# lionl1106/Clip-Neural-image-conpression

Measured on AMD Instinct MI355X. Metric: images/sec @256px 50-step DDIM, batch=8/GPU, higher is better.
Workload: dtype bf16; 1 GPU; 256px base=128 ch_mult=(1, 2, 2) 50-step DDIM (eta=0), batch=8/GPU, key-seeded synthetic weights (out.* x0.1), synthetic z / x_T; global_batch=8, parallelism=dp1 (independent batches, no collective in the loop), graph=hipGraph, one replay per step, steps_in_flight=1

## Files before the change

clip-neural-image-conpression_amd/csrc/ccn_api.hip:

```cpp
#include "../../include/ccn_hip.h"
#include "ccn_internal.h"

#include <algorithm>
#include <cmath>
#include <cstdio>
#include <cstdlib>
#include <cstring>
#include <functional>
#include <map>
#include <memory>
#include <string>
#include <vector>

using namespace ccn;

namespace {

thread_local std::string g_err;
int fail(int code, const std::string& msg) { g_err = msg; return code; }
#define HIPCHK(expr)                                                                                     \
    do {                                                                                                 \
        hipError_t e_ = (expr);                                                                          \
        if (e_ != hipSuccess)                                                                            \
            return fail(CCN_EHIP, std::string(#expr) + ": " + hipGetErrorString(e_));                    \
// ... 87 lines not shown
    std::vector<int32_t> ts;
    std::vector<float> coef;
    std::vector<float> sigma;
    const float* noise = nullptr;
    hipGraph_t graph = nullptr;
    hipGraphExec_t exec = nullptr;
};

struct RouteRec {
    std::string name;
    int kind = 0;
    const char* kernel = "";
    int th = 0, ksplit = 1, n_nt = 1;
    const char* gn = "none";
    bool film = false, res = false;
    int ops = -1;
};

constexpr size_t kMaxGraphsPerPlan = 4;
struct Plan {
    int B = 0, H = 0, W = 0, steps = 0;
    void* ws = nullptr;
    size_t bytes = 0;
    int32_t* ts_dev = nullptr;
    float *temb = nullptr, *t1 = nullptr, *tp = nullptr, *zp = nullptr, *film = nullptr;
    float *zbuf = nullptr, *xstate = nullptr;
    std::vector<std::pair<void*, size_t>> zero_once;
    unsigned* counters = nullptr;
    int n_counters = 0;
    std::vector<int32_t> ts_keep;
    std::vector<Launch> ops;
    std::map<std::string, TensorRef> named;
    std::vector<RouteRec> routes;
    std::vector<GraphEntry> graphs;
    ~Plan() {
        for (auto& g : graphs) {
            if (g.exec) (void)hipGraphExecDestroy(g.exec);
            if (g.graph) (void)hipGraphDestroy(g.graph);
        }
    }
};

}

struct ccn_handle_s {
// ... 346 lines not shown
        a.in = in.p; a.w = cw.w; a.wfrag = r.uses_frag() ? cw.wfrag : nullptr; a.bias = cw.bias; a.out = out.p;
        a.film = nullptr; a.res = res ? res->p : nullptr;
        a.ops = cw.split ? 1 : 0; a.wscale_inv = cw.inv_scale;
        RouteRec rec;
        if (h->split) rec.ops = a.ops;
        rec.kind = cw.kind; rec.th = r.th; rec.ksplit = r.ksplit; rec.n_nt = r.n_nt; rec.film = film_off >= 0; rec.res = res != nullptr;
        rec.gn = gn_ab ? "prologue" : "none";
        static const bool no_instat = diag_env("CCN_NO_INSTAT") != nullptr;
        if (in_norm) {
            const int G_in = groups_for(cw.Cin), cpg_in = cw.Cin / G_in;
            if (r.gs_ok && !no_instat && in.C == cw.Cin && conv_in_kernel_stats(h->cfg.dtype, in.C, G_in, in.n_sp, in.bn)) {
                a.gs_part = in.part; a.gs_gamma = in_norm->gamma; a.gs_beta = in_norm->beta;
                a.gs_inv_count = 1.0 / ((double)cpg_in * in.H * in.W);
                a.gs_nsp = in.n_sp; a.gs_nnt = in.n_nt; a.gs_bn = in.bn; a.gs_cpg = cpg_in;
                rec.gn = "instat";
            } else { gn_ab = gn(in, *in_norm); rec.gn = "prologue"; }
        }
        a.gn_ab = gn_ab;
        rec.kernel = conv_kernel_name(conv_kernel_for(cw.kind, cw.BN, a));
        plan->routes.push_back(rec);
        if (r.ksplit == 2) {
            a.kpart = bump.take((size_t)B * g.Hout * g.Wout * cw.Cout * h->elem);
            const size_t fbytes = (size_t)B * r.fin_blocks * 4 * sizeof(unsigned);
            a.kflag = (unsigned*)bump.take(fbytes);
            if (a.kflag) plan->zero_once.push_back({a.kflag, fbytes});
        }
        a.film_bstride = film_stride;
        a.err = h->err_dev;
        if (want_part) {
            out.part = (float2*)bump.take((size_t)B * a.G * a.nslot * sizeof(float2));
            out.n_sp = r.part_nsp; out.n_nt = r.part_nnt; out.bn = r.part_bn;
// ... 88 lines not shown
        return o;
    }

    TensorRef resblock(const ResW& r, const TensorRef& x, bool out_feeds_gn, int film_off = -2)
    {
        static const bool preact_pr = diag_env("CCN_PREACT_PR") != nullptr;
        const bool pre = conv_wants_preact(r.c1.kind, r.c1.BN, r.c1.Cout_pad / r.c1.BN) && r.C / (h->elem == 2 ? 8 : 4) <= 256 &&
                         (preact_pr || r.c1.Cout_pad / r.c1.BN >= 6 || !route(r.c1, x.H, x.W, false, false, false).pr);
        static const bool fuse_act = !diag_env("CCN_NO_FUSED_GNACT");
        const bool f1 = pre && fuse_act && x.n_sp > 0, f2 = pre && fuse_act;
        TensorRef y = new_tensor(r.C, x.H, x.W);
        if (f1) { TensorRef xa = preact_fused(x, r.n1); conv(r.c1, F_C3S1, xa, y, nullptr, film_off == -2 ? r.film_off : film_off, nullptr, true); }
        else if (pre) {
            const float2* ab1 = gn(x, r.n1);
            TensorRef xa = preact(x, ab1); conv(r.c1, F_C3S1, xa, y, nullptr, film_off == -2 ? r.film_off : film_off, nullptr, true);
        } else conv(r.c1, F_C3S1, x, y, nullptr, film_off == -2 ? r.film_off : film_off, nullptr, true, false, false, &r.n1);
        label(r.prefix + ".film", f1 ? "preact_fused" : (pre ? "preact" : nullptr));
        plan->named[r.prefix + ".film"] = y;
        TensorRef o = new_tensor(r.C, x.H, x.W);
        if (f2) { TensorRef ya = preact_fused(y, r.n2); conv(r.c2, F_C3S1, ya, o, nullptr, -1, &x, out_feeds_gn); }
        else if (pre) {
            const float2* ab2 = gn(y, r.n2);
            TensorRef ya = preact(y, ab2); conv(r.c2, F_C3S1, ya, o, nullptr, -1, &x, out_feeds_gn);
        } else conv(r.c2, F_C3S1, y, o, nullptr, -1, &x, out_feeds_gn, false, false, &r.n2);
        label(r.prefix, f2 ? "preact_fused" : (pre ? "preact" : nullptr));
        plan->named[r.prefix] = o;
        return o;
    }
};

int build_plan(ccn_handle_s* h, Plan* plan, void* ws, bool measure)
{
    const ccn_config_t& c = h->cfg;
    PlanBuilder pb(h, plan, ws, measure);
    const int B = plan->B, H = plan->H, W = plan->W, S = plan->steps;
    const int TR = B > S ? B : S, FR = S * B > B ? S * B : B;
    plan->ts_dev = (int32_t*)pb.bump.take((size_t)S * 4);
    plan->temb = (float*)pb.bump.take((size_t)TR * c.time_dim * 4);
    plan->t1 = (float*)pb.bump.take((size_t)TR * c.time_dim * 4 * 4);
    plan->tp = (float*)pb.bump.take((size_t)TR * c.time_dim * 4);
    plan->zp = (float*)pb.bump.take((size_t)B * c.time_dim * 4);
    plan->film = (float*)pb.bump.take((size_t)FR * h->F * 4);
    plan->zbuf = (float*)pb.bump.take((size_t)B * c.z_dim * 4);
    plan->xstate = (float*)pb.bump.take((size_t)B * c.img_ch * H * W * 4);
    plan->counters = (unsigned*)pb.bump.take((size_t)kMaxNorms * B * 4);
    plan->n_counters = 0;

    plan->ops.clear(); plan->named.clear(); plan->routes.clear();
    TensorRef img; img.C = c.img_ch; img.H = H; img.W = W;
    TensorRef x;
    std::vector<TensorRef> skips;
    const size_t nl = h->layers.size();
    for (size_t li = 0; li < nl; ++li) {
        const Layer& L = h->layers[li];
        const bool next_is_gn = li + 1 < nl && (h->layers[li + 1].type == L_RES || h->layers[li + 1].type == L_HEAD);
        switch (L.type) {
            case L_STEM: {
                x = pb.new_tensor(h->stem.Cout, H, W);
                pb.conv(h->stem, F_STEM, img, x, nullptr, -1, nullptr, next_is_gn, true, false);
                pb.label(L.name);
                plan->named[L.name] = x;
                break;
            }
// ... 18 lines not shown
                TensorRef sk = skips.back(); skips.pop_back();
                if (sk.C != cw.Cout || sk.H != o.H || sk.W != o.W) return fail(CCN_EINVAL, "skip shape mismatch");
                pb.conv(cw, F_CT4, x, o, nullptr, -1, &sk, next_is_gn);
                pb.label(L.name);
                plan->named[L.name] = o;
                x = o;
                break;
            }
            case L_HEAD: {
                static const bool no_head2 = diag_env("CCN_NO_HEAD2") != nullptr;
                if (!no_head2 && head2_supported(c.dtype, h->head.Cin, h->head.Cout, h->G)) {
                    std::shared_ptr<ConvArgs> ap(new ConvArgs());
                    ConvArgs& a = *ap;
                    a.in = x.p; a.bias = h->head.bias; a.B = B; a.Hin = H; a.Win = W; a.Cin = h->head.Cin; a.Cout = h->head.Cout;
                    a.Hout = H; a.Wout = W;
                    const float2* ab = pb.gn(x, h->out_norm);
                    void* scratch = pb.bump.take(head2_scratch_bytes(B, x.C));
                    const float* wf = h->head_w_f32;
                    const double macs = (double)B * H * W * h->head.Cout * 9.0 * h->head.Cin;
                    Launch Lh{F_HEAD, 2.0 * macs, ((double)B * H * W * x.C + 9.0 * x.C * h->head.Cout) * h->elem + 3.0 * (double)B * H * W * h->head.Cout * 4, nullptr};
                    Lh.fn = [=](hipStream_t s, const StepCtx& sc) -> hipError_t {
                        ConvArgs k = *ap;
                        k.x_state = sc.x_state; k.eps_out = sc.eps_out; k.do_ddim = sc.do_ddim;
                        k.c0 = sc.c[0]; k.c1 = sc.c[1]; k.c2 = sc.c[2]; k.c3 = sc.c[3];
                        k.noise = sc.noise; k.sigma = sc.sigma;
                        return launch_head2(k, ab, wf, scratch, sc.step, s);
                    };
                    plan->ops.push_back(std::move(Lh));
                    RouteRec rec;
                    rec.name = L.name; rec.kind = KIND_HEAD; rec.kernel = "head2"; rec.th = 8; rec.gn = "weights";
                    if (h->split) rec.ops = 0;
                    plan->routes.push_back(rec);
                    break;
                }
                const float2* ab = pb.gn(x, h->out_norm);
                TensorRef none;
                pb.conv(h->head, F_HEAD, x, none, ab, -1, nullptr, false, false, true);
                pb.label(L.name);
                break;
            }
        }
    }
    plan->bytes = align_up(pb.bump.off, 256);
    return CCN_OK;
}

void drop_plans(ccn_handle_s* h, size_t keep_newest)
{
    if (h->plans.size() <= keep_newest) return;
    (void)hipDeviceSynchronize();
    while (h->plans.size() > keep_newest) h->plans.erase(h->plans.begin());
}

// ... 55 lines not shown
    if (h->profiling) {
        int rc = ensure_events(h, h->ev_used + 2);
        if (rc) return rc;
        const int e0 = (int)h->ev_used, e1 = e0 + 1;
        h->ev_used += 2;
        HIPCHK(hipEventRecord(h->ev_pool[e0], s));
        HIPCHK(L.fn(s, c));
        HIPCHK(hipEventRecord(h->ev_pool[e1], s));
        h->recs.push_back({L.family, L.flops, L.bytes, e0, e1});
        return CCN_OK;
    }
    HIPCHK(L.fn(s, c));
    return CCN_OK;
}

int run_conditioning(ccn_handle_s* h, Plan* p, hipStream_t s, const int64_t* t_i64, int TR, int FR, int a_div)
{
    const ccn_config_t& c = h->cfg;
    const int td = c.time_dim, B = p->B;
    std::vector<Launch> v;
    const float* z = p->zbuf;
    v.push_back({F_COND, 0, 0, [=](hipStream_t st, const StepCtx&) {
        return t_i64 ? launch_temb_i64(t_i64, p->temb, TR, td, st) : launch_temb_i32(p->ts_dev, p->temb, TR, td, st); }});
    v.push_back({F_COND, 2.0 * TR * td * 4.0 * td, 0, [=](hipStream_t st, const StepCtx&) {
        return launch_linear(p->temb, nullptr, 1, TR, h->tp0_w, h->tp0_b, p->t1, TR, td, 4 * td, 1, st); }});
    v.push_back({F_COND, 2.0 * TR * td * 4.0 * td, 0, [=](hipStream_t st, const StepCtx&) {
        return launch_linear(p->t1, nullptr, 1, TR, h->tp2_w, h->tp2_b, p->tp, TR, 4 * td, td, 0, st); }});
    v.push_back({F_COND, 2.0 * B * c.z_dim * td, 0, [=](hipStream_t st, const StepCtx&) {
        return launch_linear(z, nullptr, 1, B, h->zp_w, h->zp_b, p->zp, B, c.z_dim, td, 1, st); }});
    v.push_back({F_COND, 2.0 * FR * td * (double)h->F, 0, [=](hipStream_t st, const StepCtx&) {
        return launch_linear(p->tp, p->zp, a_div, B, h->film_w, h->film_b, p->film, FR, td, h->F, 0, st); }});
    StepCtx c0;
    for (auto& L : v) { int rc = run_launch(h, L, s, c0); if (rc) return rc; }
    return CCN_OK;
}

int run_steps(ccn_handle_s* h, Plan* p, hipStream_t s, int steps, const float* coef, const float* sigma = nullptr, const float* noise = nullptr)
{
    const size_t img = (size_t)p->B * h->cfg.img_ch * p->H * p->W;
    for (int i = 0; i < steps; ++i) {
        StepCtx c;
        c.step = i; c.x_in = p->xstate; c.x_state = p->xstate; c.eps_out = nullptr; c.do_ddim = 1;
        for (int k = 0; k < 4; ++k) c.c[k] = coef[i * 4 + k];
        if (sigma && noise && sigma[i] > 0.f) { c.noise = noise + (size_t)i * img; c.sigma = sigma[i]; }
        for (auto& L : p->ops) { int rc = run_launch(h, L, s, c); if (rc) return rc; }
    }
// ... 240 lines not shown
    if (rc) return rc;
    *bytes = p.bytes;
    return CCN_OK;
}

int ccn_forward(ccn_handle_t h, const float* x_dev, const float* z_dev, const int64_t* t_dev, float* eps_dev,
                int32_t B, int32_t H, int32_t W, void* workspace_dev, size_t workspace_bytes, void* stream)
{
    int rc = check_ready(h);
    if (rc) return rc;
    if (!x_dev || !z_dev || !t_dev || !eps_dev) return fail(CCN_EINVAL, "null tensor pointer");
    Plan* p = nullptr;
    if ((rc = get_plan(h, B, H, W, 1, workspace_dev, workspace_bytes, &p))) return rc;
    hipStream_t s = (hipStream_t)stream;
    HIPCHK(hipMemcpyAsync(p->zbuf, z_dev, (size_t)B * h->cfg.z_dim * 4, hipMemcpyDeviceToDevice, s));
    if ((rc = run_conditioning(h, p, s, t_dev, B, B, 1))) return rc;
    StepCtx c;
    c.step = 0; c.x_in = x_dev; c.x_state = nullptr; c.eps_out = eps_dev; c.do_ddim = 0;
    for (auto& L : p->ops) if ((rc = run_launch(h, L, s, c))) return rc;
    return CCN_OK;
}

static int sample_impl(ccn_handle_t h, const float* z_dev, const float* x_T_dev, float* x_out_dev, int32_t B, int32_t H, int32_t W,
                       int32_t steps, const int32_t* ts_host, const float* coef_host, const float* sigma_host, const float* noise_dev,
                       void* workspace_dev, size_t workspace_bytes, void* stream, int32_t use_graph)
{
    int rc = check_ready(h);
    if (rc) return rc;
    if (!z_dev || !x_T_dev || !x_out_dev || !ts_host || !coef_host) return fail(CCN_EINVAL, "null pointer");
    Plan* p = nullptr;
    if ((rc = get_plan(h, B, H, W, steps, workspace_dev, workspace_bytes, &p))) return rc;
    hipStream_t s = (hipStream_t)stream;
    const size_t img_bytes = (size_t)B * h->cfg.img_ch * H * W * 4;
    HIPCHK(hipMemcpyAsync(p->zbuf, z_dev, (size_t)B * h->cfg.z_dim * 4, hipMemcpyDeviceToDevice, s));
    if (x_T_dev != p->xstate) HIPCHK(hipMemcpyAsync(p->xstate, x_T_dev, img_bytes, hipMemcpyDeviceToDevice, s));

    if (p->ts_keep.size() != (size_t)steps || std::memcmp(p->ts_keep.data(), ts_host, (size_t)steps * 4)) {
        HIPCHK(hipStreamSynchronize(s));
        p->ts_keep.assign(ts_host, ts_host + steps);
        HIPCHK(hipMemcpy(p->ts_dev, p->ts_keep.data(), (size_t)steps * 4, hipMemcpyHostToDevice));
    }
    if (use_graph && !h->profiling) {
        GraphEntry* ge = nullptr;
        for (auto& g : p->graphs)
            if (g.steps == steps && !std::memcmp(g.ts.data(), ts_host, (size_t)steps * 4) &&
                !std::memcmp(g.coef.data(), coef_host, (size_t)steps * 16) && g.noise == noise_dev &&
                g.sigma.size() == (sigma_host ? (size_t)steps : 0) &&
                (!sigma_host || !std::memcmp(g.sigma.data(), sigma_host, (size_t)steps * 4))) { ge = &g; break; }
        if (!ge) {
            GraphEntry g;
            g.steps = steps; g.ts.assign(ts_host, ts_host + steps); g.coef.assign(coef_host, coef_host + steps * 4);
            if (sigma_host) g.sigma.assign(sigma_host, sigma_host + steps);
            g.noise = noise_dev;
            HIPCHK(hipStreamBeginCapture(h->cap_stream, hipStreamCaptureModeRelaxed));
            rc = run_conditioning(h, p, h->cap_stream, nullptr, steps, steps * B, B);
            if (!rc) rc = run_steps(h, p, h->cap_stream, steps, coef_host, sigma_host, noise_dev);
            hipGraph_t graph = nullptr;
            const hipError_t ce = hipStreamEndCapture(h->cap_stream, &graph);
            if (rc) { if (graph) (void)hipGraphDestroy(graph); return rc; }
            if (ce != hipSuccess) return fail(CCN_EHIP, std::string("hipStreamEndCapture: ") + hipGetErrorString(ce));
            g.graph = graph;
            HIPCHK(hipGraphInstantiate(&g.exec, g.graph, nullptr, nullptr, 0));
            if (p->graphs.size() >= kMaxGraphsPerPlan) {
                HIPCHK(hipDeviceSynchronize());
                GraphEntry& old = p->graphs.front();
                if (old.exec) (void)hipGraphExecDestroy(old.exec);
                if (old.graph) (void)hipGraphDestroy(old.graph);
                p->graphs.erase(p->graphs.begin());
            }
            p->graphs.push_back(g);
            ge = &p->graphs.back();
        } else if (ge != &p->graphs.back()) {
            std::rotate(p->graphs.begin() + (ge - p->graphs.data()), p->graphs.begin() + (ge - p->graphs.data()) + 1, p->graphs.end());
            ge = &p->graphs.back();
        }
        HIPCHK(hipGraphLaunch(ge->exec, s));
    } else {
        if ((rc = run_conditioning(h, p, s, nullptr, steps, steps * B, B))) return rc;
        if ((rc = run_steps(h, p, s, steps, coef_host, sigma_host, noise_dev))) return rc;
    }
    if (x_out_dev != p->xstate) HIPCHK(hipMemcpyAsync(x_out_dev, p->xstate, img_bytes, hipMemcpyDeviceToDevice, s));
    return CCN_OK;
}

int ccn_sample(ccn_handle_t h, const float* z_dev, const float* x_T_dev, float* x_out_dev, int32_t B, int32_t H, int32_t W,
               int32_t steps, const int32_t* ts_host, const float* coef_host, void* workspace_dev, size_t workspace_bytes,
               void* stream, int32_t use_graph)
{
    return sample_impl(h, z_dev, x_T_dev, x_out_dev, B, H, W, steps, ts_host, coef_host, nullptr, nullptr, workspace_dev, workspace_bytes, stream, use_graph);
}

int ccn_sample_eta(ccn_handle_t h, const float* z_dev, const float* x_T_dev, float* x_out_dev, int32_t B, int32_t H, int32_t W,
                   int32_t steps, const int32_t* ts_host, const float* coef_host, const float* sigma_host, const float* noise_dev,
// ... 102 lines not shown
    const TensorRef& t = it->second;
    if (out_elems < (size_t)p->B * t.C * t.H * t.W) return fail(CCN_EINVAL, "output buffer too small");
    hipStream_t s = (hipStream_t)stream;
    HIPCHK(launch_nhwc_to_nchw(h->cfg.dtype, t.p, out_dev, p->B, t.C, t.H, t.W, s));
    HIPCHK(hipStreamSynchronize(s));
    return CCN_OK;
}

extern "C" int ccn_internal_plan_routes(ccn_handle_t h, char* buf, size_t cap)
{
    if (!h || h->plans.empty()) return -1;
    static const char* kinds[] = {"C3S1", "C3S2", "CT4", "STEM", "HEAD"};
    std::string text;
    for (const RouteRec& r : h->plans.back()->routes) {
        char line[256];
        std::snprintf(line, sizeof(line), "%s %s %s th=%d ksplit=%d n_nt=%d gn=%s film=%d res=%d", r.name.c_str(), kinds[r.kind], r.kernel,
                      r.th, r.ksplit, r.n_nt, r.gn, r.film ? 1 : 0, r.res ? 1 : 0);
        text += line;
        if (r.ops >= 0) text += r.ops ? " ops=f16x3" : " ops=f32";
        text += "\n";
    }
    if (buf && cap) {
        const size_t n = std::min(text.size(), cap - 1);
        std::memcpy(buf, text.data(), n);
        buf[n] = 0;
    }
    return (int)text.size();
}

int ccn_poll_errors(ccn_handle_t h)
{
    if (!h) return fail(CCN_EINVAL, "null handle");
    return check_device_errors(h);
}

int ccn_profile_enable(ccn_handle_t h, int32_t on)
{
    if (!h) return fail(CCN_EINVAL, "null handle");
    h->profiling = on != 0;
    h->recs.clear();
    h->ev_used = 0;
    return CCN_OK;
// ... 43 lines not shown
```

clip-neural-image-conpression_amd/csrc/ccn_head.hip:

```cpp
#include "ccn_device.h"

namespace ccn {

namespace {
constexpr int HG_PITCH = 27;
constexpr int HG_ROWS = 10, HG_COLS = 34, HG_PIX = HG_ROWS * HG_COLS;
}

__global__ __launch_bounds__(512) void head_prep_kernel(const float2* __restrict__ ab, int C, const float* __restrict__ w, int Cout,
                                                         unsigned short* __restrict__ wq, float* __restrict__ sq, float* __restrict__ carry, int step)
{
    const int b = blockIdx.y, s = blockIdx.x, tid = threadIdx.x, ksteps = C / 16;
    const float* abf = (const float*)(ab + (size_t)b * C);
    const int N = Cout * 9;
    if (s < ksteps) {
        const int e = tid & 7, ln = tid >> 3;
        const int n = ln & 31, c = 16 * s + 8 * (ln >> 5) + e;
        float v = 0.f;
        if (n < N) { const int tap = n / Cout, co = n - tap * Cout; v = abf[4 * (c >> 1) + (c & 1)] * w[((size_t)co * C + c) * 9 + tap]; }
        const size_t ci = ((size_t)b * ksteps + s) * 512 + tid;
        const float t = v + (step > 0 ? carry[ci] : 0.f);
        const unsigned u = __float_as_uint(t);
        const unsigned hi = (u + 0x7fffu + ((u >> 16) & 1u)) & 0xffff0000u;
        carry[ci] = t - __uint_as_float(hi);
        wq[ci] = (unsigned short)(hi >> 16);
    } else {
        const int n = tid >> 4, part = tid & 15;
        float acc = 0.f;
        if (n < N) {
            const int tap = n / Cout, co = n - tap * Cout;
            for (int c = part; c < C; c += 16) acc = fmaf(abf[4 * (c >> 1) + 2 + (c & 1)], w[((size_t)co * C + c) * 9 + tap], acc);
        }
#pragma unroll
        for (int m = 1; m < 16; m <<= 1) acc += __shfl_xor(acc, m);
        if (part == 0) sq[b * 32 + n] = acc;
    }
}

template <int KSTEPS>
__global__ __launch_bounds__(256, 4) void head_kernel(const ConvArgs a, const unsigned short* __restrict__ wq, const float* __restrict__ sq,
                                                   const float* __restrict__ bias)
{
    typedef __bf16 T;
    __shared__ float Gs[HG_PIX * HG_PITCH];
    __shared__ float Ss[32];
    const int tid = threadIdx.x, lane = tid & 63, wave = tid >> 6, r = lane & 31, h = lane >> 5;
// ... 110 lines not shown
            float xn = __fadd_rn(__fmul_rn(a.c2, x0v), __fmul_rn(a.c3, e));
            if (a.noise) xn = __fadd_rn(xn, __fmul_rn(a.sigma, a.noise[idx]));
            a.x_state[idx] = xn;
        }
    }
}

bool head2_supported(int dtype, int cin, int cout, int G)
{
    const int g = cin < G ? cin : G;
    return dtype == 1 && cout * 9 <= 27 && cout <= 3 && (cin == 32 || cin == 64 || cin == 128 || cin == 192) && cin % g == 0;
}

size_t head2_scratch_bytes(int B, int C) { return (size_t)B * (C / 16) * 512 * 6 + (size_t)B * 32 * 4 + 512; }

hipError_t launch_head2(const ConvArgs& a, const float2* ab, const float* w_f32, void* scratch, int step, hipStream_t s)
{
    if ((size_t)a.B * a.Hin * a.Win * a.Cin * 2 >= 0x7FFFFFF0u || a.Cin > 512) return hipErrorInvalidValue;
    const int ks = a.Cin / 16;
    const size_t nfrag = (size_t)a.B * ks * 512;
    unsigned short* wq = (unsigned short*)scratch;
    float* carry = (float*)((char*)scratch + ((nfrag * 2 + 255) & ~(size_t)255));
    float* sq = carry + nfrag;
    hipLaunchKernelGGL(head_prep_kernel, dim3(ks + 1, a.B), dim3(512), 0, s, ab, a.Cin, w_f32, a.Cout, wq, sq, carry, step);
    const unsigned grid = (unsigned)(a.B * ((a.Hin + 7) / 8) * ((a.Win + 31) / 32));
    switch (ks) {
        case 12: hipLaunchKernelGGL(head_kernel<12>, dim3(grid), dim3(256), 0, s, a, wq, sq, a.bias); break;
        case 8: hipLaunchKernelGGL(head_kernel<8>, dim3(grid), dim3(256), 0, s, a, wq, sq, a.bias); break;
        case 4: hipLaunchKernelGGL(head_kernel<4>, dim3(grid), dim3(256), 0, s, a, wq, sq, a.bias); break;
        case 2: hipLaunchKernelGGL(head_kernel<2>, dim3(grid), dim3(256), 0, s, a, wq, sq, a.bias); break;
        default: return hipErrorInvalidValue;
    }
    return hipGetLastError();
}

}
```

clip-neural-image-conpression_amd/csrc/ccn_internal.h:

```cpp
#pragma once
#include <hip/hip_runtime.h>
#include <stdint.h>
#include <stddef.h>

#include <stdlib.h>

#ifdef CCN_DIAG
#define CCN_DBG_BIT(a, bit) ((((a).dbg) & (bit)) != 0)
#define CCN_STAMPS_PTR(a) ((a).stamps)
namespace ccn { inline const char* diag_env(const char* name) { return getenv(name); } }
#else
#define CCN_DBG_BIT(a, bit) false
#define CCN_STAMPS_PTR(a) ((unsigned long long*)nullptr)
namespace ccn { inline const char* diag_env(const char*) { return nullptr; } }
#endif

namespace ccn {

__host__ __device__ inline int pr3_slice(int g, int k32) { return ((g & 1) << 2) | (k32 << 1) | (g >> 1); }
__host__ __device__ inline size_t pr3_frag_index(int n, int k, int t, int Np)
{
    const int chunk = k >> 6, s = (k & 63) >> 3, e = k & 7;
    const int g = ((s >> 2) & 1) | ((s & 1) << 1), k32 = (s >> 1) & 1;
    const int nn = n >> 5, c = (n >> 4) & 1, lane = g * 16 + (n & 15);
// ... 140 lines not shown
struct ConvRoute {
    ConvQuery q;
    ConvGeom g;
    int th, n_nt, nchunk, ntaps, ksplit, nslot, fin_blocks;
    bool pr, stem2;
    bool gs_ok;
    int part_nsp, part_nnt, part_bn;
    bool uses_frag() const { return pr || stem2; }
    void fill(ConvArgs& a) const;
};
ConvRoute conv_route(const ConvQuery& q, const ConvPolicy& p);
bool conv_in_kernel_stats(int dtype, int C, int G, int n_sp, int bn);

bool head2_supported(int dtype, int cin, int cout, int G);
size_t head2_scratch_bytes(int B, int C);
hipError_t launch_head2(const ConvArgs& a, const float2* ab, const float* w_f32, void* scratch, int step, hipStream_t s);

bool conv_wants_preact(int kind, int bn, int n_nt);
hipError_t launch_gn_act(int dtype, const void* x, const float2* ab, void* y, int B, int HW, int C, hipStream_t s);
hipError_t launch_gn_act_fused(int dtype, const void* x, void* y, int B, int HW, int C, const float2* part, int G, int n_sp, int n_nt,
                               int bn, int cpg, double count, const float* gamma, const float* beta, float eps, hipStream_t s,
                               float2* ab_out = nullptr, float2* stats_out = nullptr);

hipError_t launch_gn_finalize(const float2* part, int B, int G, int n_sp, int n_nt, int bn, int cpg, int C,
                              double count, const float* gamma, const float* beta, float eps,
                              float2* ab, hipStream_t s);

hipError_t launch_temb_i64(const int64_t* t, float* out, int n, int dim, hipStream_t s);
hipError_t launch_temb_i32(const int32_t* t, float* out, int n, int dim, hipStream_t s);
hipError_t launch_linear(const float* xa, const float* xb, int a_div, int b_mod, const float* W, const float* b,
                         float* y, int R, int K, int N, int act_silu, hipStream_t s);

hipError_t launch_ddim_step(float* x, const float* eps, const float* noise, float c0, float c1, float c2, float c3,
                            float sigma, int64_t n, hipStream_t s);
hipError_t launch_q_sample(float* out, const float* x0, const float* noise, const float* a, const float* sg,
                           int B, int64_t per, hipStream_t s);
hipError_t launch_predict_x0(float* out, const float* xt, const float* eps, const float* a, const float* sg,
                             int B, int64_t per, hipStream_t s);
hipError_t launch_film_nchw(const float* x, const float* sc, const float* sh, float* y, int B, int C, int64_t hw,
                            hipStream_t s);
hipError_t launch_nchw_to_nhwc(int dtype, const float* src, void* dst, int B, int C, int H, int W, hipStream_t s);
hipError_t launch_nhwc_to_nchw(int dtype, const void* src, float* dst, int B, int C, int H, int W, hipStream_t s);
hipError_t launch_gn_partials(int dtype, const void* x, float2* part, int B, int HW, int C, int cpg, int G,
                              int nslot, hipStream_t s);

}
// ... 1 lines not shown
```

clip-neural-image-conpression_amd/csrc/ccn_kernels.hip:

```cpp
#include "ccn_conv_tile.h"

namespace ccn {

__host__ __device__ constexpr int cmax(int a, int b) { return a > b ? a : b; }

template <int AK, int IS> struct HaloGeom {
    static constexpr int HOFF = AK == A_NHWC ? 1 : 0;
    static constexpr int ROWS = AK == A_NHWC ? (IS == 1 ? 6 : 10) : 4;
    static constexpr int PITCH = AK == A_NHWC ? (IS == 1 ? 34 : 66) : 32;
    static constexpr int BYTES = ROWS * PITCH * 128;
};
template <int AK, int IS, int BN> struct LdsGeom {
    static constexpr int A_BYTES = HaloGeom<AK, IS>::BYTES;
    static constexpr int B_BYTES = BN * 128;
    static constexpr int TOTAL = EpiLds<4, BN, 4>::total(A_BYTES + 2 * B_BYTES);
};

template <typename T, int AK, int IS, int EPI, int WM, int WN, int MF, int NF>
__global__ __launch_bounds__(256) void conv_igemm_kernel(const ConvArgs a)
{
    static_assert(WM * WN == 4 && WM * MF == 4, "4 waves, 4 M-fragments of 32 pixels (TH=4 rows of TW=32)");
    constexpr int BN = WN * NF * 32;
    constexpr int EPC = Vec16<T>::EPC;
    constexpr int CKE = 8 * EPC;
// ... 704 lines not shown
        for (int s = 32; s >= 1; s >>= 1) acc += __shfl_xor(acc, s);
        if (lane == 0) {
            float v = acc + (bias ? bias[n] : 0.f);
            if (act_silu) v = v / (1.0f + expf(-v));
            y[(size_t)rr * N + n] = v;
        }
    }
}
hipError_t launch_linear(const float* xa, const float* xb, int a_div, int b_mod, const float* W, const float* b, float* y,
                         int R, int K, int N, int act_silu, hipStream_t s)
{
    hipLaunchKernelGGL(linear_kernel, dim3((N + 3) / 4, (R + 15) / 16), dim3(256), 0, s, xa, xb, a_div, b_mod, W, b, y, R, K, N, act_silu);
    return hipGetLastError();
}

__global__ void ddim_step_kernel(float* __restrict__ x, const float* __restrict__ eps, const float* __restrict__ noise,
                                 float c0, float c1, float c2, float c3, float sigma, int64_t n)
{
    for (int64_t i = (int64_t)blockIdx.x * blockDim.x + threadIdx.x; i < n; i += (int64_t)gridDim.x * blockDim.x) {
        const float e = eps[i];
        float x0 = __fdiv_rn(__fsub_rn(x[i], __fmul_rn(c0, e)), c1);
        x0 = fminf(fmaxf(x0, -1.0f), 1.0f);
        float xn = __fadd_rn(__fmul_rn(c2, x0), __fmul_rn(c3, e));
        if (noise) xn = __fadd_rn(xn, __fmul_rn(sigma, noise[i]));
        x[i] = xn;
    }
}
hipError_t launch_ddim_step(float* x, const float* eps, const float* noise, float c0, float c1, float c2, float c3, float sigma,
                            int64_t n, hipStream_t s)
{
// ... 93 lines not shown
```

clip-neural-image-conpression_amd/csrc/ccn_train.hip:

```cpp
#include "../../include/ccn_hip.h"
#include "ccn_train.h"

#include <climits>
#include <cmath>
#include <cstdio>
#include <cstdlib>
#include <cstring>
#include <map>
#include <string>
#include <vector>

using namespace ccn;

extern "C" void ccn_internal_set_error(const char* msg);

namespace {

int tfail(int code, const std::string& msg) { ccn_internal_set_error(msg.c_str()); return code; }
#define THIP(expr)                                                                                       \
    do {                                                                                                 \
        hipError_t e_ = (expr);                                                                          \
        if (e_ != hipSuccess) { err = std::string(#expr) + ": " + hipGetErrorString(e_); return false; } \
    } while (0)

// ... 493 lines not shown
                    x = o;
                    break;
                }
                case L_HEAD: {
                    head_in = x;
                    if (!gn_fwd(x, tr->out_norm, ab_o, st_o)) return false;
                    static const bool no_head2 = diag_env("CCN_TRAIN_NO_HEAD2") != nullptr;
                    if (!no_head2 && head2_supported(tr->cfg.dtype, tr->head.Cin, tr->head.Cout, tr->G) && (double)B * H * W * x.C * 2 < 2.0e9) {
                        void* scratch = take(head2_scratch_bytes(B, x.C));
                        if (!launch) break;
                        ConvArgs a{};
                        a.in = x.p; a.bias = par(tr->head.pb); a.B = B; a.Hin = H; a.Win = W; a.Cin = tr->head.Cin; a.Cout = tr->head.Cout;
                        a.Hout = H; a.Wout = W; a.eps_out = eps;
                        mark(TF_CONV_FWD, 2.0 * B * H * W * (double)tr->head.Cout * 9.0 * tr->head.Cin);
                        note(RN_CONV, KIND_HEAD, "head2", 1);
                        if (!ok(launch_head2(a, ab_o, par(tr->head.pw), scratch, 0, st), "head")) return false;
                        break;
                    }
                    TT none;
                    if (!run_conv(TF_CONV_FWD, fwd_route(tr->head, x.H, x.W, ab_o != nullptr, false, false), tr->head.pd_f, tr->head.pf_f,
                                  launch ? par(tr->head.pb) : nullptr, x.p, &none, nullptr, ab_o, nullptr, nullptr, false, eps)) return false;
                    break;
                }
            }
        }
        if (launch && (fwd_side_used || tr->pack_dg_pending)) {
            if (hipEventRecord(tr->pack_dg_done, tr->side) != hipSuccess || hipStreamWaitEvent(st, tr->pack_dg_done, 0) != hipSuccess) { err = "stream join failed"; return false; }
            tr->pack_dg_pending = false;
        }
        return true;
    }
// ... 497 lines not shown
```

Before: 83.96 images/sec.

## Fuse head GroupNorm finalize into prep, add row-batched linear, cache time conditioning

The output GroupNorm statistics are now finalized inside the head prep kernel from the partial sums, using double-precision cross-lane reductions, instead of a separate gn launch. Conditioning linears switch to a new row-batched kernel that keeps weights in registers and stages input rows in LDS. The time-embedding MLP is computed once per timestep schedule outside the captured graph and reused across calls, so only the FiLM part runs each replay. This cuts per-step launches and per-call conditioning work, but adds extra reduction work in every head prep block and state that must stay valid across calls.

New measurement: 84.57 images/sec (median of 6 runs). About the same (+0.7%).

```diff
diff --git a/clip-neural-image-conpression_amd/csrc/ccn_api.hip b/clip-neural-image-conpression_amd/csrc/ccn_api.hip
--- a/clip-neural-image-conpression_amd/csrc/ccn_api.hip
+++ b/clip-neural-image-conpression_amd/csrc/ccn_api.hip
@@ -125,6 +125,7 @@
     int th = 0, ksplit = 1, n_nt = 1;
     const char* gn = "none";
     bool film = false, res = false;
+    int fin = 0;
     int ops = -1;
 };
 
@@ -140,6 +141,8 @@
     unsigned* counters = nullptr;
     int n_counters = 0;
     std::vector<int32_t> ts_keep;
+    int small_variant = 1;
+    bool tp_ready = false;
     std::vector<Launch> ops;
     std::map<std::string, TensorRef> named;
     std::vector<RouteRec> routes;
@@ -516,7 +519,7 @@
                 a.gs_inv_count = 1.0 / ((double)cpg_in * in.H * in.W);
                 a.gs_nsp = in.n_sp; a.gs_nnt = in.n_nt; a.gs_bn = in.bn; a.gs_cpg = cpg_in;
                 rec.gn = "instat";
-            } else { gn_ab = gn(in, *in_norm); rec.gn = "prologue"; }
+            } else { gn_ab = gn(in, *in_norm); rec.gn = "prologue"; rec.fin = 1; }
         }
         a.gn_ab = gn_ab;
         rec.kernel = conv_kernel_name(conv_kernel_for(cw.kind, cw.BN, a));
@@ -635,6 +638,7 @@
         else if (pre) {
             const float2* ab1 = gn(x, r.n1);
             TensorRef xa = preact(x, ab1); conv(r.c1, F_C3S1, xa, y, nullptr, film_off == -2 ? r.film_off : film_off, nullptr, true);
+            plan->routes.back().fin = 1;
         } else conv(r.c1, F_C3S1, x, y, nullptr, film_off == -2 ? r.film_off : film_off, nullptr, true, false, false, &r.n1);
         label(r.prefix + ".film", f1 ? "preact_fused" : (pre ? "preact" : nullptr));
         plan->named[r.prefix + ".film"] = y;
@@ -643,6 +647,7 @@
         else if (pre) {
             const float2* ab2 = gn(y, r.n2);
             TensorRef ya = preact(y, ab2); conv(r.c2, F_C3S1, ya, o, nullptr, -1, &x, out_feeds_gn);
+            plan->routes.back().fin = 1;
         } else conv(r.c2, F_C3S1, y, o, nullptr, -1, &x, out_feeds_gn, false, false, &r.n2);
         label(r.prefix, f2 ? "preact_fused" : (pre ? "preact" : nullptr));
         plan->named[r.prefix] = o;
@@ -668,6 +673,8 @@
     plan->n_counters = 0;
 
     plan->ops.clear(); plan->named.clear(); plan->routes.clear();
+    plan->small_variant = small_launch_variant();
+    plan->tp_ready = false;
     TensorRef img; img.C = c.img_ch; img.H = H; img.W = W;
     TensorRef x;
     std::vector<TensorRef> skips;
@@ -716,7 +723,13 @@
                     ConvArgs& a = *ap;
                     a.in = x.p; a.bias = h->head.bias; a.B = B; a.Hin = H; a.Win = W; a.Cin = h->head.Cin; a.Cout = h->head.Cout;
                     a.Hout = H; a.Wout = W;
-                    const float2* ab = pb.gn(x, h->out_norm);
+                    HeadNorm hn;
+                    const float2* ab = nullptr;
+                    const bool fin_in_prep = plan->small_variant != 0 && x.n_sp > 0;
+                    if (fin_in_prep) {
+                        hn.part = x.part; hn.G = pb.groups_for(x.C); hn.cpg = x.C / hn.G; hn.n_sp = x.n_sp; hn.n_nt = x.n_nt; hn.bn = x.bn;
+                        hn.count = (double)hn.cpg * x.H * x.W; hn.gamma = h->out_norm.gamma; hn.beta = h->out_norm.beta;
+                    } else ab = pb.gn(x, h->out_norm);
                     void* scratch = pb.bump.take(head2_scratch_bytes(B, x.C));
                     const float* wf = h->head_w_f32;
                     const double macs = (double)B * H * W * h->head.Cout * 9.0 * h->head.Cin;
@@ -726,11 +739,12 @@
                         k.x_state = sc.x_state; k.eps_out = sc.eps_out; k.do_ddim = sc.do_ddim;
                         k.c0 = sc.c[0]; k.c1 = sc.c[1]; k.c2 = sc.c[2]; k.c3 = sc.c[3];
                         k.noise = sc.noise; k.sigma = sc.sigma;
-                        return launch_head2(k, ab, wf, scratch, sc.step, s);
+                        return launch_head2(k, ab, hn, wf, scratch, sc.step, s);
                     };
                     plan->ops.push_back(std::move(Lh));
                     RouteRec rec;
                     rec.name = L.name; rec.kind = KIND_HEAD; rec.kernel = "head2"; rec.th = 8; rec.gn = "weights";
+                    rec.fin = fin_in_prep ? 0 : 1;
                     if (h->split) rec.ops = 0;
                     plan->routes.push_back(rec);
                     break;
@@ -739,6 +753,7 @@
                 TensorRef none;
                 pb.conv(h->head, F_HEAD, x, none, ab, -1, nullptr, false, false, true);
                 pb.label(L.name);
+                plan->routes.back().fin = 1;
                 break;
             }
         }
@@ -824,22 +839,28 @@
     return CCN_OK;
 }
 
-int run_conditioning(ccn_handle_s* h, Plan* p, hipStream_t s, const int64_t* t_i64, int TR, int FR, int a_div)
+enum { COND_TIME = 1, COND_FILM = 2 };
+int run_conditioning(ccn_handle_s* h, Plan* p, hipStream_t s, const int64_t* t_i64, int TR, int FR, int a_div, int parts)
 {
     const ccn_config_t& c = h->cfg;
     const int td = c.time_dim, B = p->B;
+    const auto linear = p->small_variant ? launch_linear_rows : launch_linear;
     std::vector<Launch> v;
     const float* z = p->zbuf;
-    v.push_back({F_COND, 0, 0, [=](hipStream_t st, const StepCtx&) {
-        return t_i64 ? launch_temb_i64(t_i64, p->temb, TR, td, st) : launch_temb_i32(p->ts_dev, p->temb, TR, td, st); }});
-    v.push_back({F_COND, 2.0 * TR * td * 4.0 * td, 0, [=](hipStream_t st, const StepCtx&) {
-        return launch_linear(p->temb, nullptr, 1, TR, h->tp0_w, h->tp0_b, p->t1, TR, td, 4 * td, 1, st); }});
-    v.push_back({F_COND, 2.0 * TR * td * 4.0 * td, 0, [=](hipStream_t st, const StepCtx&) {
-        return launch_linear(p->t1, nullptr, 1, TR, h->tp2_w, h->tp2_b, p->tp, TR, 4 * td, td, 0, st); }});
-    v.push_back({F_COND, 2.0 * B * c.z_dim * td, 0, [=](hipStream_t st, const StepCtx&) {
-        return launch_linear(z, nullptr, 1, B, h->zp_w, h->zp_b, p->zp, B, c.z_dim, td, 1, st); }});
-    v.push_back({F_COND, 2.0 * FR * td * (double)h->F, 0, [=](hipStream_t st, const StepCtx&) {
-        return launch_linear(p->tp, p->zp, a_div, B, h->film_w, h->film_b, p->film, FR, td, h->F, 0, st); }});
+    if (parts & COND_TIME) {
+        v.push_back({F_COND, 0, 0, [=](hipStream_t st, const StepCtx&) {
+            return t_i64 ? launch_temb_i64(t_i64, p->temb, TR, td, st) : launch_temb_i32(p->ts_dev, p->temb, TR, td, st); }});
+        v.push_back({F_COND, 2.0 * TR * td * 4.0 * td, 0, [=](hipStream_t st, const StepCtx&) {
+            return linear(p->temb, nullptr, 1, TR, h->tp0_w, h->tp0_b, p->t1, TR, td, 4 * td, 1, st); }});
+        v.push_back({F_COND, 2.0 * TR * td * 4.0 * td, 0, [=](hipStream_t st, const StepCtx&) {
+            return linear(p->t1, nullptr, 1, TR, h->tp2_w, h->tp2_b, p->tp, TR, 4 * td, td, 0, st); }});
+    }
+    if (parts & COND_FILM) {
+        v.push_back({F_COND, 2.0 * B * c.z_dim * td, 0, [=](hipStream_t st, const StepCtx&) {
+            return linear(z, nullptr, 1, B, h->zp_w, h->zp_b, p->zp, B, c.z_dim, td, 1, st); }});
+        v.push_back({F_COND, 2.0 * FR * td * (double)h->F, 0, [=](hipStream_t st, const StepCtx&) {
+            return linear(p->tp, p->zp, a_div, B, h->film_w, h->film_b, p->film, FR, td, h->F, 0, st); }});
+    }
     StepCtx c0;
     for (auto& L : v) { int rc = run_launch(h, L, s, c0); if (rc) return rc; }
     return CCN_OK;
@@ -1110,7 +1131,8 @@
     if ((rc = get_plan(h, B, H, W, 1, workspace_dev, workspace_bytes, &p))) return rc;
     hipStream_t s = (hipStream_t)stream;
     HIPCHK(hipMemcpyAsync(p->zbuf, z_dev, (size_t)B * h->cfg.z_dim * 4, hipMemcpyDeviceToDevice, s));
-    if ((rc = run_conditioning(h, p, s, t_dev, B, B, 1))) return rc;
+    p->tp_ready = false;
+    if ((rc = run_conditioning(h, p, s, t_dev, B, B, 1, COND_TIME | COND_FILM))) return rc;
     StepCtx c;
     c.step = 0; c.x_in = x_dev; c.x_state = nullptr; c.eps_out = eps_dev; c.do_ddim = 0;
     for (auto& L : p->ops) if ((rc = run_launch(h, L, s, c))) return rc;
@@ -1135,6 +1157,15 @@
         HIPCHK(hipStreamSynchronize(s));
         p->ts_keep.assign(ts_host, ts_host + steps);
         HIPCHK(hipMemcpy(p->ts_dev, p->ts_keep.data(), (size_t)steps * 4, hipMemcpyHostToDevice));
+        p->tp_ready = false;
+    }
+    int cond_parts = COND_TIME | COND_FILM;
+    if (p->small_variant) {
+        if (!p->tp_ready) {
+            if ((rc = run_conditioning(h, p, s, nullptr, steps, steps * B, B, COND_TIME))) return rc;
+            p->tp_ready = true;
+        }
+        cond_parts = COND_FILM;
     }
     if (use_graph && !h->profiling) {
         GraphEntry* ge = nullptr;
@@ -1149,7 +1180,7 @@
             if (sigma_host) g.sigma.assign(sigma_host, sigma_host + steps);
             g.noise = noise_dev;
             HIPCHK(hipStreamBeginCapture(h->cap_stream, hipStreamCaptureModeRelaxed));
-            rc = run_conditioning(h, p, h->cap_stream, nullptr, steps, steps * B, B);
+            rc = run_conditioning(h, p, h->cap_stream, nullptr, steps, steps * B, B, cond_parts);
             if (!rc) rc = run_steps(h, p, h->cap_stream, steps, coef_host, sigma_host, noise_dev);
             hipGraph_t graph = nullptr;
             const hipError_t ce = hipStreamEndCapture(h->cap_stream, &graph);
@@ -1172,7 +1203,7 @@
         }
         HIPCHK(hipGraphLaunch(ge->exec, s));
     } else {
-        if ((rc = run_conditioning(h, p, s, nullptr, steps, steps * B, B))) return rc;
+        if ((rc = run_conditioning(h, p, s, nullptr, steps, steps * B, B, cond_parts))) return rc;
         if ((rc = run_steps(h, p, s, steps, coef_host, sigma_host, noise_dev))) return rc;
     }
     if (x_out_dev != p->xstate) HIPCHK(hipMemcpyAsync(x_out_dev, p->xstate, img_bytes, hipMemcpyDeviceToDevice, s));
@@ -1305,8 +1336,8 @@
     std::string text;
     for (const RouteRec& r : h->plans.back()->routes) {
         char line[256];
-        std::snprintf(line, sizeof(line), "%s %s %s th=%d ksplit=%d n_nt=%d gn=%s film=%d res=%d", r.name.c_str(), kinds[r.kind], r.kernel,
-                      r.th, r.ksplit, r.n_nt, r.gn, r.film ? 1 : 0, r.res ? 1 : 0);
+        std::snprintf(line, sizeof(line), "%s %s %s th=%d ksplit=%d n_nt=%d gn=%s film=%d res=%d fin=%d", r.name.c_str(), kinds[r.kind], r.kernel,
+                      r.th, r.ksplit, r.n_nt, r.gn, r.film ? 1 : 0, r.res ? 1 : 0, r.fin);
         text += line;
         if (r.ops >= 0) text += r.ops ? " ops=f16x3" : " ops=f32";
         text += "\n";
@@ -1317,6 +1348,17 @@
         buf[n] = 0;
     }
     return (int)text.size();
+}
+
+extern "C" long ccn_internal_read_film(ccn_handle_t h, float* out_dev, size_t out_elems, void* stream)
+{
+    if (!h || h->plans.empty()) return -1;
+    const Plan* p = h->plans.back().get();
+    const size_t n = (size_t)p->steps * p->B * h->F;
+    if (!out_dev || out_elems < n) return -1;
+    hipStream_t s = (hipStream_t)stream;
+    if (hipMemcpyAsync(out_dev, p->film, n * 4, hipMemcpyDeviceToDevice, s) != hipSuccess || hipStreamSynchronize(s) != hipSuccess) return -1;
+    return (long)n;
 }
 
 int ccn_poll_errors(ccn_handle_t h)
diff --git a/clip-neural-image-conpression_amd/csrc/ccn_head.hip b/clip-neural-image-conpression_amd/csrc/ccn_head.hip
--- a/clip-neural-image-conpression_amd/csrc/ccn_head.hip
+++ b/clip-neural-image-conpression_amd/csrc/ccn_head.hip
@@ -7,17 +7,104 @@
 constexpr int HG_ROWS = 10, HG_COLS = 34, HG_PIX = HG_ROWS * HG_COLS;
 }
 
-__global__ __launch_bounds__(512) void head_prep_kernel(const float2* __restrict__ ab, int C, const float* __restrict__ w, int Cout,
+__device__ __forceinline__ void swap32_f64(double& a, double& b)
+{
+    const uint2 ua = __builtin_bit_cast(uint2, a), ub = __builtin_bit_cast(uint2, b);
+    const auto lo = __builtin_amdgcn_permlane32_swap(ua.x, ub.x, false, false), hi = __builtin_amdgcn_permlane32_swap(ua.y, ub.y, false, false);
+    a = __builtin_bit_cast(double, make_uint2(lo[0], hi[0])); b = __builtin_bit_cast(double, make_uint2(lo[1], hi[1]));
+}
+__device__ __forceinline__ void swap16_f64(double& a, double& b)
+{
+    const uint2 ua = __builtin_bit_cast(uint2, a), ub = __builtin_bit_cast(uint2, b);
+    const auto lo = __builtin_amdgcn_permlane16_swap(ua.x, ub.x, false, false), hi = __builtin_amdgcn_permlane16_swap(ua.y, ub.y, false, false);
+    a = __builtin_bit_cast(double, make_uint2(lo[0], hi[0])); b = __builtin_bit_cast(double, make_uint2(lo[1], hi[1]));
+}
+template <int S> __device__ __forceinline__ double row_ror_f64(double v)
+{
+    const uint2 u = __builtin_bit_cast(uint2, v);
+    return __builtin_bit_cast(double, make_uint2(__builtin_amdgcn_update_dpp(0u, u.x, 0x120 + S, 0xf, 0xf, false),
+                                                 __builtin_amdgcn_update_dpp(0u, u.y, 0x120 + S, 0xf, 0xf, false)));
+}
+__device__ __forceinline__ double butterfly4_f64(double q0, double q1, double q2, double q3)
+{
+    swap32_f64(q0, q1); swap32_f64(q2, q3);
+    double t01 = q0 + q1, t23 = q2 + q3;
+    swap16_f64(t01, t23);
+    double u = t01 + t23;
+    u += row_ror_f64<8>(u);
+    u += row_ror_f64<4>(u);
+    u += row_ror_f64<2>(u);
+    u += row_ror_f64<1>(u);
+    return u;
+}
+
+__global__ __launch_bounds__(512) void head_prep_kernel(const float2* __restrict__ ab, const HeadNorm hn, int C, const float* __restrict__ w, int Cout,
                                                          unsigned short* __restrict__ wq, float* __restrict__ sq, float* __restrict__ carry, int step)
 {
+    constexpr int GW = 4, GR = 8 * GW;
+    __shared__ double red[GR][4][2];
+    __shared__ float sc_s[512], sh_s[512];
     const int b = blockIdx.y, s = blockIdx.x, tid = threadIdx.x, ksteps = C / 16;
-    const float* abf = (const float*)(ab + (size_t)b * C);
+    if (hn.part) {
+        const int lane = tid & 63, wave = tid >> 6;
+        for (int g0 = 0; g0 < hn.G; g0 += GR) {
+            const int ng = min(GR, hn.G - g0);
+            double s1[GW][4], s2[GW][4];
+#pragma unroll
+            for (int gi = 0; gi < GW; ++gi) {
+                const int g = g0 + wave + 8 * gi;
+#pragma unroll
+                for (int q = 0; q < 4; ++q) { s1[gi][q] = 0.0; s2[gi][q] = 0.0; }
+                if (wave + 8 * gi >= ng) continue;
+                const int jlo = (g * hn.cpg) / hn.bn, jhi = ((g + 1) * hn.cpg - 1) / hn.bn, nj = jhi - jlo + 1, ne = hn.n_sp * nj;
+                const float2* base = hn.part + (size_t)(b * hn.G + g) * hn.n_sp * hn.n_nt;
+                for (int e0 = 0; e0 < ne; e0 += 256) {
+#pragma unroll
+                    for (int q = 0; q < 4; ++q) {
+                        const int e = e0 + 64 * q + lane;
+                        if (e < ne) {
+                            const int sp = e / nj, j = jlo + (e - sp * nj);
+                            const float2 v = base[(size_t)sp * hn.n_nt + j];
+                            s1[gi][q] += (double)v.x; s2[gi][q] += (double)v.y;
+                        }
+                    }
+                }
+            }
+#pragma unroll
+            for (int gi = 0; gi < GW; ++gi) {
+                if (wave + 8 * gi >= ng) continue;
+                const double r1 = butterfly4_f64(s1[gi][0], s1[gi][1], s1[gi][2], s1[gi][3]);
+                const double r2 = butterfly4_f64(s2[gi][0], s2[gi][1], s2[gi][2], s2[gi][3]);
+                if ((lane & 15) == 0) {
+                    const int q = ((lane >> 5) & 1) | (((lane >> 4) & 1) << 1);
+                    red[wave + 8 * gi][q][0] = r1; red[wave + 8 * gi][q][1] = r2;
+                }
+            }
+            __syncthreads();
+            for (int c = g0 * hn.cpg + tid; c < (g0 + ng) * hn.cpg; c += 512) {
+                const int gl = c / hn.cpg - g0;
+                const double t1 = (red[gl][0][0] + red[gl][1][0]) + (red[gl][2][0] + red[gl][3][0]);
+                const double t2 = (red[gl][0][1] + red[gl][1][1]) + (red[gl][2][1] + red[gl][3][1]);
+                const double mean = t1 / hn.count;
+                double var = t2 / hn.count - mean * mean;
+                if (var < 0.0) var = 0.0;
+                const double rstd = 1.0 / sqrt(var + (double)hn.eps);
+                const double sc = (double)hn.gamma[c] * rstd;
+                sc_s[c] = (float)sc; sh_s[c] = (float)((double)hn.beta[c] - mean * sc);
+            }
+            __syncthreads();
+        }
+    } else {
+        const float* abf = (const float*)(ab + (size_t)b * C);
+        for (int c = tid; c < C; c += 512) { sc_s[c] = abf[4 * (c >> 1) + (c & 1)]; sh_s[c] = abf[4 * (c >> 1) + 2 + (c & 1)]; }
+        __syncthreads();
+    }
     const int N = Cout * 9;
     if (s < ksteps) {
         const int e = tid & 7, ln = tid >> 3;
         const int n = ln & 31, c = 16 * s + 8 * (ln >> 5) + e;
         float v = 0.f;
-        if (n < N) { const int tap = n / Cout, co = n - tap * Cout; v = abf[4 * (c >> 1) + (c & 1)] * w[((size_t)co * C + c) * 9 + tap]; }
+        if (n < N) { const int tap = n / Cout, co = n - tap * Cout; v = sc_s[c] * w[((size_t)co * C + c) * 9 + tap]; }
         const size_t ci = ((size_t)b * ksteps + s) * 512 + tid;
         const float t = v + (step > 0 ? carry[ci] : 0.f);
         const unsigned u = __float_as_uint(t);
@@ -29,7 +116,7 @@
         float acc = 0.f;
         if (n < N) {
             const int tap = n / Cout, co = n - tap * Cout;
-            for (int c = part; c < C; c += 16) acc = fmaf(abf[4 * (c >> 1) + 2 + (c & 1)], w[((size_t)co * C + c) * 9 + tap], acc);
+            for (int c = part; c < C; c += 16) acc = fmaf(sh_s[c], w[((size_t)co * C + c) * 9 + tap], acc);
         }
 #pragma unroll
         for (int m = 1; m < 16; m <<= 1) acc += __shfl_xor(acc, m);
@@ -170,15 +257,16 @@
 
 size_t head2_scratch_bytes(int B, int C) { return (size_t)B * (C / 16) * 512 * 6 + (size_t)B * 32 * 4 + 512; }
 
-hipError_t launch_head2(const ConvArgs& a, const float2* ab, const float* w_f32, void* scratch, int step, hipStream_t s)
+hipError_t launch_head2(const ConvArgs& a, const float2* ab, const HeadNorm& hn, const float* w_f32, void* scratch, int step, hipStream_t s)
 {
     if ((size_t)a.B * a.Hin * a.Win * a.Cin * 2 >= 0x7FFFFFF0u || a.Cin > 512) return hipErrorInvalidValue;
+    if (hn.part ? (hn.G <= 0 || hn.cpg <= 0 || hn.G * hn.cpg != a.Cin || hn.bn <= 0 || hn.n_sp <= 0 || hn.n_nt <= 0) : ab == nullptr) return hipErrorInvalidValue;
     const int ks = a.Cin / 16;
     const size_t nfrag = (size_t)a.B * ks * 512;
     unsigned short* wq = (unsigned short*)scratch;
     float* carry = (float*)((char*)scratch + ((nfrag * 2 + 255) & ~(size_t)255));
     float* sq = carry + nfrag;
-    hipLaunchKernelGGL(head_prep_kernel, dim3(ks + 1, a.B), dim3(512), 0, s, ab, a.Cin, w_f32, a.Cout, wq, sq, carry, step);
+    hipLaunchKernelGGL(head_prep_kernel, dim3(ks + 1, a.B), dim3(512), 0, s, ab, hn, a.Cin, w_f32, a.Cout, wq, sq, carry, step);
     const unsigned grid = (unsigned)(a.B * ((a.Hin + 7) / 8) * ((a.Win + 31) / 32));
     switch (ks) {
         case 12: hipLaunchKernelGGL(head_kernel<12>, dim3(grid), dim3(256), 0, s, a, wq, sq, a.bias); break;
diff --git a/clip-neural-image-conpression_amd/csrc/ccn_internal.h b/clip-neural-image-conpression_amd/csrc/ccn_internal.h
--- a/clip-neural-image-conpression_amd/csrc/ccn_internal.h
+++ b/clip-neural-image-conpression_amd/csrc/ccn_internal.h
@@ -178,7 +178,14 @@
 
 bool head2_supported(int dtype, int cin, int cout, int G);
 size_t head2_scratch_bytes(int B, int C);
-hipError_t launch_head2(const ConvArgs& a, const float2* ab, const float* w_f32, void* scratch, int step, hipStream_t s);
+struct HeadNorm {
+    const float2* part = nullptr;
+    int G = 0, n_sp = 0, n_nt = 0, bn = 0, cpg = 0;
+    double count = 0.0;
+    const float* gamma = nullptr; const float* beta = nullptr;
+    float eps = 1e-5f;
+};
+hipError_t launch_head2(const ConvArgs& a, const float2* ab, const HeadNorm& hn, const float* w_f32, void* scratch, int step, hipStream_t s);
 
 bool conv_wants_preact(int kind, int bn, int n_nt);
 hipError_t launch_gn_act(int dtype, const void* x, const float2* ab, void* y, int B, int HW, int C, hipStream_t s);
@@ -194,6 +201,9 @@
 hipError_t launch_temb_i32(const int32_t* t, float* out, int n, int dim, hipStream_t s);
 hipError_t launch_linear(const float* xa, const float* xb, int a_div, int b_mod, const float* W, const float* b,
                          float* y, int R, int K, int N, int act_silu, hipStream_t s);
+hipError_t launch_linear_rows(const float* xa, const float* xb, int a_div, int b_mod, const float* W, const float* b,
+                              float* y, int R, int K, int N, int act_silu, hipStream_t s);
+int small_launch_variant();
 
 hipError_t launch_ddim_step(float* x, const float* eps, const float* noise, float c0, float c1, float c2, float c3,
                             float sigma, int64_t n, hipStream_t s);
diff --git a/clip-neural-image-conpression_amd/csrc/ccn_kernels.hip b/clip-neural-image-conpression_amd/csrc/ccn_kernels.hip
--- a/clip-neural-image-conpression_amd/csrc/ccn_kernels.hip
+++ b/clip-neural-image-conpression_amd/csrc/ccn_kernels.hip
@@ -742,6 +742,170 @@
     return hipGetLastError();
 }
 
+constexpr int LIN_COLS = 4, LIN_WAVES = 4, LIN_LDS_FLOATS = 8192;
+template <int S> __device__ __forceinline__ float lin_row_ror(float u)
+{
+    return __uint_as_float(__builtin_amdgcn_update_dpp(0u, __float_as_uint(u), 0x120 + S, 0xf, 0xf, false));
+}
+__device__ __forceinline__ float lin_butterfly4(const float (&acc)[4])
+{
+    const auto s01 = __builtin_amdgcn_permlane32_swap(__float_as_uint(acc[0]), __float_as_uint(acc[1]), false, false);
+    const auto s23 = __builtin_amdgcn_permlane32_swap(__float_as_uint(acc[2]), __float_as_uint(acc[3]), false, false);
+    const float t01 = __uint_as_float(s01[0]) + __uint_as_float(s01[1]);
+    const float t23 = __uint_as_float(s23[0]) + __uint_as_float(s23[1]);
+    const auto sq = __builtin_amdgcn_permlane16_swap(__float_as_uint(t01), __float_as_uint(t23), false, false);
+    float u = __uint_as_float(sq[0]) + __uint_as_float(sq[1]);
+    u += lin_row_ror<8>(u);
+    u += lin_row_ror<4>(u);
+    u += lin_row_ror<2>(u);
+    u += lin_row_ror<1>(u);
+    return u;
+}
+template <int KJ, bool FULL, bool VEC>
+__global__ __launch_bounds__(256) void linear_rows_kernel(const float* __restrict__ xa, const float* __restrict__ xb, int a_div, int b_mod,
+                                                           const float* __restrict__ W, const float* __restrict__ bias, float* __restrict__ y,
+                                                           int R, int K, int N, int act_silu, int rows_per_block)
+{
+    __shared__ __attribute__((aligned(16))) float xs[LIN_LDS_FLOATS];
+    constexpr int KP = KJ * 64;
+    const int tid = threadIdx.x, lane = tid & 63, wave = tid >> 6;
+    const int n0 = (blockIdx.x * LIN_WAVES + wave) * LIN_COLS;
+    float w[LIN_COLS][KJ];
+#pragma unroll
+    for (int c = 0; c < LIN_COLS; ++c)
+#pragma unroll
+        for (int j = 0; j < KJ; ++j) {
+            const int k = lane + 64 * j;
+            w[c][j] = (n0 + c < N && (FULL || k < K)) ? W[(size_t)(n0 + c) * K + k] : 0.f;
+        }
+    const int my_n = n0 + (((lane >> 5) & 1) | (((lane >> 4) & 1) << 1));
+    const bool writer = (lane & 15) == 0 && my_n < N;
+    const float bv = (bias && writer) ? bias[my_n] : 0.f;
+    const int r_begin = blockIdx.y * rows_per_block, r_end = min(R, r_begin + rows_per_block);
+    constexpr int RC = LIN_LDS_FLOATS / KP;
+    constexpr int U = 4;
+    for (int rc0 = r_begin; rc0 < r_end; rc0 += RC) {
+        const int nr = min(RC, r_end - rc0);
+        __syncthreads();
+        if constexpr (VEC) {
+            constexpr int QP = KP / 4;
+            const int total = nr * QP;
+            for (int i0 = tid; i0 < total; i0 += 256 * U) {
+                f32x4 va[U], vb[U];
+#pragma unroll
+                for (int u = 0; u < U; ++u) {
+                    const int i = i0 + 256 * u, rr = i / QP, k = (i - rr * QP) * 4, row = rc0 + rr;
+                    va[u] = f32x4{0.f, 0.f, 0.f, 0.f}; vb[u] = va[u];
+                    if (i < total) {
+                        va[u] = *(const f32x4*)(xa + (size_t)(row / a_div) * K + k);
+                        if (xb) vb[u] = *(const f32x4*)(xb + (size_t)(row % b_mod) * K + k);
+                    }
+                }
+#pragma unroll
+                for (int u = 0; u < U; ++u) {
+                    const int i = i0 + 256 * u;
+                    if (i < total) {
+                        f32x4 v = va[u];
+                        if (xb) { v[0] += vb[u][0]; v[1] += vb[u][1]; v[2] += vb[u][2]; v[3] += vb[u][3]; }
+                        *(f32x4*)(xs + 4 * i) = v;
+                    }
+                }
+            }
+        } else {
+            const int total = nr * KP;
+            for (int i0 = tid; i0 < total; i0 += 256 * U) {
+                float va[U], vb[U];
+#pragma unroll
+                for (int u = 0; u < U; ++u) {
+                    const int i = i0 + 256 * u, rr = i / KP, k = i - rr * KP, row = rc0 + rr;
+                    va[u] = 0.f; vb[u] = 0.f;
+                    if (i < total && (FULL || k < K)) {
+                        va[u] = xa[(size_t)(row / a_div) * K + k];
+                        if (xb) vb[u] = xb[(size_t)(row % b_mod) * K + k];
+                    }
+                }
+#pragma unroll
+                for (int u = 0; u < U; ++u) {
+                    const int i = i0 + 256 * u;
+                    if (i < total) xs[i] = xb ? va[u] + vb[u] : va[u];
+                }
+            }
+        }
+        __syncthreads();
+        if (n0 >= N) continue;
+        for (int rr = 0; rr < nr; rr += 2) {
+            const bool two = rr + 1 < nr;
+            const float* x0 = xs + rr * KP + lane;
+            const float* x1 = two ? x0 + KP : x0;
+            float acc[2][LIN_COLS];
+#pragma unroll
+            for (int c = 0; c < LIN_COLS; ++c) { acc[0][c] = 0.f; acc[1][c] = 0.f; }
+#pragma unroll
+            for (int j = 0; j < KJ; ++j) {
+                const float xv0 = x0[64 * j], xv1 = x1[64 * j];
+                if (FULL || lane + 64 * j < K) {
+#pragma unroll
+                    for (int c = 0; c < LIN_COLS; ++c) { acc[0][c] = fmaf(xv0, w[c][j], acc[0][c]); acc[1][c] = fmaf(xv1, w[c][j], acc[1][c]); }
+                }
+            }
+            const float u0 = lin_butterfly4(acc[0]), u1 = lin_butterfly4(acc[1]);
+            if (writer) {
+                float v0 = u0 + bv, v1 = u1 + bv;
+                if (act_silu) { v0 = v0 / (1.0f + expf(-v0)); v1 = v1 / (1.0f + expf(-v1)); }
+                y[(size_t)(rc0 + rr) * N + my_n] = v0;
+                if (two) y[(size_t)(rc0 + rr + 1) * N + my_n] = v1;
+            }
+        }
+    }
+}
+
+template <int KJ>
+static hipError_t launch_linear_rows_kj(const float* xa, const float* xb, int a_div, int b_mod, const float* W, const float* b, float* y,
+                                        int R, int K, int N, int act_silu, hipStream_t s)
+{
+    const int gx = (N + LIN_COLS * LIN_WAVES - 1) / (LIN_COLS * LIN_WAVES);
+    int gy = (8192 + gx - 1) / gx;
+    const int max_gy = (R + 15) / 16;
+    if (gy > max_gy) gy = max_gy;
+    if (gy < 1) gy = 1;
+    const int rpb = (R + gy - 1) / gy;
+    gy = (R + rpb - 1) / rpb;
+    const dim3 grid(gx, gy);
+    const bool vec = K == KJ * 64 && (((uintptr_t)xa | (uintptr_t)xb) & 15) == 0;
+    if (vec)
+        hipLaunchKernelGGL((linear_rows_kernel<KJ, true, true>), grid, dim3(256), 0, s, xa, xb, a_div, b_mod, W, b, y, R, K, N, act_silu, rpb);
+    else if (K == KJ * 64)
+        hipLaunchKernelGGL((linear_rows_kernel<KJ, true, false>), grid, dim3(256), 0, s, xa, xb, a_div, b_mod, W, b, y, R, K, N, act_silu, rpb);
+    else
+        hipLaunchKernelGGL((linear_rows_kernel<KJ, false, false>), grid, dim3(256), 0, s, xa, xb, a_div, b_mod, W, b, y, R, K, N, act_silu, rpb);
+    return hipGetLastError();
+}
+
+hipError_t launch_linear_rows(const float* xa, const float* xb, int a_div, int b_mod, const float* W, const float* b, float* y,
+                              int R, int K, int N, int act_silu, hipStream_t s)
+{
+    if (R <= 0 || K <= 0 || N <= 0 || a_div <= 0 || b_mod <= 0) return hipErrorInvalidValue;
+    const int kj = (K + 63) / 64;
+    if (kj <= 1) return launch_linear_rows_kj<1>(xa, xb, a_div, b_mod, W, b, y, R, K, N, act_silu, s);
+    if (kj <= 2) return launch_linear_rows_kj<2>(xa, xb, a_div, b_mod, W, b, y, R, K, N, act_silu, s);
+    if (kj <= 4) return launch_linear_rows_kj<4>(xa, xb, a_div, b_mod, W, b, y, R, K, N, act_silu, s);
+    if (kj <= 8) return launch_linear_rows_kj<8>(xa, xb, a_div, b_mod, W, b, y, R, K, N, act_silu, s);
+    if (kj <= 16) return launch_linear_rows_kj<16>(xa, xb, a_div, b_mod, W, b, y, R, K, N, act_silu, s);
+    return launch_linear(xa, xb, a_div, b_mod, W, b, y, R, K, N, act_silu, s);
+}
+
+static int g_small_launch_variant = 1;
+int small_launch_variant() { return g_small_launch_variant; }
+extern "C" int ccn_internal_set_small_launch_variant(int v) { const int old = g_small_launch_variant; g_small_launch_variant = v ? 1 : 0; return old; }
+
+extern "C" int ccn_internal_linear(int variant, const float* xa, const float* xb, int a_div, int b_mod, const float* W, const float* bias,
+                                   float* y, int R, int K, int N, int act_silu, void* stream)
+{
+    const hipError_t e = variant ? launch_linear_rows(xa, xb, a_div, b_mod, W, bias, y, R, K, N, act_silu, (hipStream_t)stream)
+                                 : launch_linear(xa, xb, a_div, b_mod, W, bias, y, R, K, N, act_silu, (hipStream_t)stream);
+    return e == hipSuccess ? 0 : (int)e;
+}
+
 __global__ void ddim_step_kernel(float* __restrict__ x, const float* __restrict__ eps, const float* __restrict__ noise,
                                  float c0, float c1, float c2, float c3, float sigma, int64_t n)
 {
diff --git a/clip-neural-image-conpression_amd/csrc/ccn_train.hip b/clip-neural-image-conpression_amd/csrc/ccn_train.hip
--- a/clip-neural-image-conpression_amd/csrc/ccn_train.hip
+++ b/clip-neural-image-conpression_amd/csrc/ccn_train.hip
@@ -531,7 +531,7 @@
                         a.Hout = H; a.Wout = W; a.eps_out = eps;
                         mark(TF_CONV_FWD, 2.0 * B * H * W * (double)tr->head.Cout * 9.0 * tr->head.Cin);
                         note(RN_CONV, KIND_HEAD, "head2", 1);
-                        if (!ok(launch_head2(a, ab_o, par(tr->head.pw), scratch, 0, st), "head")) return false;
+                        if (!ok(launch_head2(a, ab_o, HeadNorm{}, par(tr->head.pw), scratch, 0, st), "head")) return false;
                         break;
                     }
                     TT none;
```
